# lyd405121/ti-raytrace

Measured on AMD Instinct MI355X. Metric: Mrays/s (primary+secondary) at 1024² 100k-tri, 1/2/4/8 GPU + HBM GB/s, higher is better.
Workload: dtype f32

## Files before the change

### ti_raytrace_amd/csrc/tirt_api.hip

```cpp
#include "tirt_internal.h"
#include "tirt_spectral.h"
#include "tirt_multi_hit.h"
#include <stddef.h>
#include <algorithm>
#include <mutex>
#include <string.h>

namespace tirt {

static thread_local std::string g_error;
void set_error(const std::string &msg) { g_error = msg; }

SceneView scene_view(const tirt_ctx *c)
{
    SceneView s;
    s.vertex = c->vertex.as<float>(); s.primitive = c->primitive.as<int>(); s.material = c->material.as<float>();
    s.shape = c->shape.as<float>(); s.light = c->light.as<int>(); s.env = c->env.as<int>();
    s.mat_lrgb = c->mat_lrgb.as<float>(); s.shade_rec = c->shade_rec.as<float4>(); s.light_rec = c->light_rec.as<float4>();
    s.tex = c->tex_count > 0 ? c->tex.as<int>() : nullptr;
    s.n = c->n; s.light_count = c->light_count; s.env_w = c->env_w; s.env_h = c->env_h; s.env_power = c->env_power;
    return s;
}
BvhView bvh_view(const tirt_ctx *c)
{
// ... 443 lines not shown
    }
    if (!strcmp(name, "plan_batches")) { TIRT_REQUIRE(value >= 0.0 && value <= 64.0, "plan_batches: 0 (automatic) .. 64"); if (flush_pending(c)) return TIRT_ERR_HIP; c->plan_nb = (int)value; return TIRT_OK; }
    if (!strcmp(name, "plan_lanes")) { TIRT_REQUIRE(value >= 0.0 && value <= TIRT_MAX_LANES, "plan_lanes: 0 (automatic) .. the lane count"); if (flush_pending(c)) return TIRT_ERR_HIP; c->plan_lanes = (int)value; return TIRT_OK; }
    if (!strcmp(name, "job_frames")) { TIRT_REQUIRE(value >= 0.0 && value <= 1.0e9, "job_frames out of range"); c->job_frames = (long)value; return TIRT_OK; }
    if (!strcmp(name, "merge_paths")) { TIRT_REQUIRE(value >= 0.0 && value <= 1.0e9, "merge_paths out of range"); c->merge_paths = (size_t)value; c->merge_user = true; return TIRT_OK; }
    if (!strcmp(name, "batch_paths")) {
        TIRT_REQUIRE(value >= 1.0 && value <= 1.0e9, "tirt_set_option: batch_paths out of range");
        c->batch_paths = (size_t)value; c->batch_user = true; return TIRT_OK;
    }
    if (!strcmp(name, "trace_lds_depth")) {
        TIRT_REQUIRE(value >= 12 && value <= 64, "trace_lds_depth: 12..64");
        TIRT_REQUIRE(trace_lds_bytes((int)value) <= c->lds_optin, "trace_lds_depth: stacks + tree top exceed the LDS a block can have on this device");
        c->tr_lds_depth = (int)value; return TIRT_OK;
    }
    if (!strcmp(name, "bdpt_stack_size")) { TIRT_REQUIRE(value >= 16 && value <= 4096, "bdpt_stack_size: 16..4096"); c->bdpt_stack = (int)value; return TIRT_OK; }
    if (!strcmp(name, "trace_timeline")) { c->timeline_arm = (int)value; c->timeline_waves = 0; return TIRT_OK; }
    if (!strcmp(name, "trace_refill_min")) { TIRT_REQUIRE(value >= 1 && value <= 64, "trace_refill_min: 1..64"); c->tr_refill_min = (int)value; return TIRT_OK; }
    if (!strcmp(name, "trace_node_min")) { TIRT_REQUIRE(value >= 1 && value <= 64, "trace_node_min: 1..64"); c->tr_node_min = (int)value; return TIRT_OK; }
    if (!strcmp(name, "bdpt_bounded")) { c->bdpt_bounded = value != 0.0 ? 1 : 0; return TIRT_OK; }
    if (!strcmp(name, "bdpt_state_fill")) { TIRT_REQUIRE(value == 0.0 || value == 1.0 || value == 2.0, "bdpt_state_fill: 0 (none), 1 (zeros) or 2 (poison)"); c->bdpt_state_fill = (int)value; return TIRT_OK; }
    if (!strcmp(name, "primary_beams")) { TIRT_REQUIRE(value == 0.0 || value == 1.0, "primary_beams: 0 or 1"); if (flush_pending(c)) return TIRT_ERR_HIP; c->primary_beams = (int)value; return TIRT_OK; }
    if (!strcmp(name, "primary_beams_rebuild")) { if (flush_pending(c)) return TIRT_ERR_HIP; c->pvb_valid = false; return TIRT_OK; }
    if (!strcmp(name, "primary_beams_diag")) { if (flush_pending(c)) return TIRT_ERR_HIP; c->pvb_diag = value != 0.0; return TIRT_OK; }
    if (!strcmp(name, "primary_beams_min_frames")) { TIRT_REQUIRE(value >= 1.0 && value <= 1.0e6, "primary_beams_min_frames out of range"); if (flush_pending(c)) return TIRT_ERR_HIP; c->primary_beams_min_frames = (int)value; return TIRT_OK; }
    if (!strcmp(name, "bdpt_lanes")) { TIRT_REQUIRE(value >= 1.0 && value <= 4.0, "bdpt_lanes: 1..4"); if (sync_all(c)) return TIRT_ERR_HIP; c->bdpt_lanes = (int)value; return TIRT_OK; }
    if (!strcmp(name, "bdpt_batch_items")) { TIRT_REQUIRE(value >= 1.0 && value <= 1.0e9, "bdpt_batch_items out of range"); c->bdpt_batch_items = (size_t)value; return TIRT_OK; }
    if (!strcmp(name, "bdpt_mem_budget")) { TIRT_REQUIRE(value >= 0, "bdpt_mem_budget: bytes >= 0"); c->bdpt_mem_budget = (size_t)value; return TIRT_OK; }
    if (!strcmp(name, "trace_slices")) {
        const int iv = (int)value;
        TIRT_REQUIRE(iv >= 1 && iv <= 64 && (iv & (iv - 1)) == 0, "trace_slices: power of two, 1..64");
        int l = 0; while ((1 << l) < iv) l++;
        c->tr_slice_log2 = l; return TIRT_OK;
    }
    if (!strcmp(name, "shade_specialize")) { TIRT_REQUIRE(value == 0.0 || value == 1.0, "shade_specialize: 0 (generic kernel) or 1"); if (flush_pending(c)) return TIRT_ERR_HIP; c->shade_specialize = (int)value; return TIRT_OK; }
    if (!strcmp(name, "shade_grid")) { TIRT_REQUIRE(value >= 1 && value <= 65536, "shade_grid: 1..65536"); c->sh_grid = (int)value; c->grid_user = true; return TIRT_OK; }
    if (!strcmp(name, "path_order_blocks")) { c->path_order_blocks = value != 0.0; return TIRT_OK; }
    if (!strcmp(name, "slices_contiguous")) { c->slices_contiguous = value != 0.0; return TIRT_OK; }
    if (!strcmp(name, "trace_grid_alone")) { TIRT_REQUIRE(value >= 1 && value <= 16384, "trace_grid_alone: 1..16384"); c->tr_grid_alone = (int)value; return TIRT_OK; }
    if (!strcmp(name, "query_chunk_rays")) {
        TIRT_REQUIRE(value >= 256.0 && value <= (double)(1 << 27), "query_chunk_rays: 256 .. 2^27");
        c->query_chunk = (size_t)value; return TIRT_OK;
    }
    if (!strcmp(name, "trace_grid")) { TIRT_REQUIRE(value >= 1 && value <= 16384, "trace_grid: 1..16384"); c->tr_grid = (int)value; c->grid_user = true; return TIRT_OK; }
    set_error(std::string("tirt_set_option: unknown option ") + name);
    return TIRT_ERR_ARG;
}
// ... 957 lines not shown
```

### ti_raytrace_amd/csrc/tirt_internal.h

```cpp
#pragma once
#include <hip/hip_runtime.h>
#include <stdint.h>
#include <stdio.h>
#include <initializer_list>
#include <string>
#include <type_traits>
#include <vector>
#include "../../include/tirt.h"
#include "tirt_device.h"

namespace tirt {

void set_error(const std::string &msg);

#define TIRT_HIP(call)                                                                          \
    do {                                                                                        \
        hipError_t e__ = (call);                                                                \
        if (e__ != hipSuccess) {                                                                \
            tirt::set_error(std::string(#call) + ": " + hipGetErrorString(e__));                \
            return TIRT_ERR_HIP;                                                                \
        }                                                                                       \
    } while (0)

#define TIRT_REQUIRE(cond, msg)                                                                 \
// ... 257 lines not shown
    long job_frames = 0;
    struct { bool valid = false; uint32_t begin = 0; int count = 0; uint32_t seed = 0; int max_depth = 0, stack_size = 0, flags = 0; bool spectral = false; } pend;
    int tr_lds_depth = 16, tr_refill_min = 18, tr_node_min = 38, tr_grid = 1280, tr_slice_log2 = 5, sh_grid = 1024;
    int path_order_blocks = 1, slices_contiguous = 0;
    int tr_grid_alone = 1280;
    tirt::DevBuf counters_mem, spill;
    int cu_count = 256;

    tirt::DevBuf bdpt_px;
    struct BdLane { tirt::DevBuf items, state, rays, hits, qidx, ctr, rad; hipEvent_t delta_done = nullptr, film_done = nullptr; } bd[4];
    int bdpt_lanes = 2;
    int bdpt_state_fill = 0;
    size_t bdpt_batch_items = (size_t)16 << 20;
    size_t bdpt_mem_budget = 0;
    int bdpt_stack = 64;
    int bdpt_bounded = 1;

    struct PvbKey { tirt::CameraView cam; unsigned long long build; int W, H, tile_rank, tile_count, tile_size, tile_blocked, P; } pvb_key;
    bool pvb_valid = false; int primary_beams = 1, primary_beams_min_frames = 16;
    unsigned long long build_serial = 0;
    struct PvbSet { tirt::DevBuf count, cand, bound; hipEvent_t busy = nullptr; } pvb_set[2];
    int pvb_cur = 0;
    int pvb_diag = 0;
    std::vector<std::pair<hipEvent_t, hipEvent_t>> pvb_ev;
    unsigned long long pvb_builds = 0, pvb_build_ns = 0, pvb_skipped = 0;
    tirt::DevBuf pvb_stat, pvb_tmp;

    tirt::DevBuf spec_dev;
    tirt::DevBuf spec_mem; bool spec_set = false; void *spec_view = nullptr;

    tirt::DevBuf trace_stage;
    tirt::DevBuf debug_mem;
    tirt::DevBuf query_mem; size_t query_chunk = (size_t)1 << 21;
    hipEvent_t query_ev_in = nullptr, query_ev_out = nullptr;
    tirt::DevBuf sd_tab, sd_state; bool sd_tab_valid = false, sd_tab_checked = false; int sd_tab_stack = 0;
    tirt::DevBuf dyn_mem;

    void *comm = nullptr; int comm_rank = 0, comm_size = 0;

    tirt::DevBuf dev_counters;
    double ms_build = 0, ms_render = 0, ms_trace_closest = 0, ms_trace_shadow = 0, ms_shade = 0;
    uint64_t launches_trace_closest = 0, launches_trace_shadow = 0, launches_shade = 0;
    bool time_kernels = false;
    std::vector<std::pair<hipEvent_t, hipEvent_t>> ev_pool;
};

// ... 148 lines not shown
```

### ti_raytrace_amd/csrc/tirt_pvb.hip

```cpp
#include "tirt_trace.h"
#include <cstring>

namespace tirt {

constexpr int PVB_CMAX = 24;
constexpr int PVB_STACK = 96;
constexpr float PVB_WIDEN = 0.55f;
constexpr float PVB_REACH = 1.5f;
constexpr int PVB_BLOCK = 1024;

struct PvbView { const int *count; const int2 *cand; const float *bound; };

__global__ void k_pvb_probes(CameraView cam, TileMap tm, int P, float4 *rays)
{
    const int k = blockIdx.x * blockDim.x + threadIdx.x;
    if (k >= P) return;
    const int p = local_to_pixel(tm, k), i = p / tm.H, j = p - i * tm.H;
    for (int pr = 0; pr < 5; pr++) {
        const float jx = pr == 0 ? 0.0f : (((pr - 1) & 1) ? 0.5f : -0.5f), jy = pr == 0 ? 0.0f : (((pr - 1) & 2) ? 0.5f : -0.5f);
        const v3 d = camera_ray_direction(cam, i, j, jx, jy);
        const size_t r = (size_t)pr * P + k;
        rays[2 * r] = make_float4(cam.eye[0], cam.eye[1], cam.eye[2], d.x);
        rays[2 * r + 1] = make_float4(d.y, d.z, 0.0f, 0.0f);
    }
}

TD float h2f(unsigned h) { return (float)__builtin_bit_cast(_Float16, (unsigned short)h); }

__global__ __launch_bounds__(64) void k_pvb_beam(BvhView b, CameraView cam, TileMap tm, int P, const float4 *probe_hits, int *count, int2 *cand, float *bound_out,
                                                 unsigned long long *stat)
{
    __shared__ int s_stack[PVB_STACK];
    __shared__ int2 s_list[PVB_CMAX * 64];
    const int lane = threadIdx.x, k = blockIdx.x * 64 + lane;
// ... 113 lines not shown
        }
        for (int a = 0; a < n; a++) cand[(size_t)a * P + k] = s_list[a * 64 + lane];
    }
    if (live) { count[k] = whole ? n : -1; bound_out[k] = bound; }
    if (stat) {
        const unsigned long long m = __ballot(whole);
        unsigned long long sm = whole ? (unsigned long long)n : 0ull;
        for (int o = 32; o > 0; o >>= 1) sm += __shfl_down(sm, o, 64);
        const unsigned long long mb = __ballot(whole && bound < INF_VALUE);
        if (lane == 0) { atomicAdd(&stat[0], (unsigned long long)__popcll(m)); atomicAdd(&stat[1], sm); atomicAdd(&stat[2], (unsigned long long)__popcll(mb)); }
    }
}

__global__ __launch_bounds__(PVB_BLOCK) void k_pvb_cand(BvhView b, PvbView pv, const float *dx, const float *dy, const float *dz, v3 eye, TileMap tm, int P, int S,
                                                  float4 *hit, int *fb_count, int *fb_slot, float *fb_dx, float *fb_dy, float *fb_dz, DevCounters *ctr,
                                                  unsigned long long *stat, unsigned long long *diag)
{
    const int s = blockIdx.x * blockDim.x + threadIdx.x, lane = threadIdx.x & 63;
    const bool live = s < S;
    int k = 0;
    if (tm.F > 0) { const int ch = __builtin_amdgcn_readfirstlane(s >> 6); k = ((ch / tm.F) << 6) | (s & 63); }
    else if (live) { int f; slot_to_frame_pixel(tm, P, s, f, k); }
    const v3 d = live ? V(__builtin_nontemporal_load(&dx[s]), __builtin_nontemporal_load(&dy[s]), __builtin_nontemporal_load(&dz[s])) : V(0.0f, 0.0f, 1.0f);
    const RayCtx r = make_ray(eye, d);
    const bool par = ray_has_parallel_axis(r);
    int n = live ? pv.count[k] : 0;
    const float bound = live ? pv.bound[k] : 0.0f;
    bool resolved = live && n >= 0;
    bool dead = false;
    if (live) {
        float tn;
        if (b.root_qcode >= 0 && !slabs(r, b.root_min[0], b.root_min[1], b.root_min[2], b.root_max[0], b.root_max[1], b.root_max[2], tn)) dead = true;
        if (!((d.x == d.x) & (d.y == d.y) & (d.z == d.z))) dead = true;
    }
    if (dead) { n = 0; resolved = true; }
    if (!resolved) n = 0;
    float hit_t = INF_VALUE, hit_u = 0.0f, hit_v = 0.0f; int hit_prim = -1, hit_leaf = -1;
    int steps = 0, trips = 0;
    for (int c = 0; c < PVB_CMAX; c++) {
        int2 en = make_int2(0, 0x7f800000);
        if (c < n) en = pv.cand[(size_t)c * P + k];
        const bool go = c < n && __int_as_float(en.y) <= hit_t;
        if (!go) n = 0;
        if (__ballot(go) == 0ull) break;
        trips++; if (go) steps++;
        if (go) (void)trace_leaf_step<true>(b, r, par, ~en.x, hit_t, hit_u, hit_v, hit_prim, hit_leaf);
    }
    if (resolved && !dead && !(hit_t <= bound) && bound < INF_VALUE) resolved = false;
    if (resolved) {
        typedef float f4n __attribute__((ext_vector_type(4)));
        f4n hv = {hit_t, hit_u, hit_v, __int_as_float(hit_prim)};
        __builtin_nontemporal_store(hv, (f4n *)&hit[s]);
    }
    const bool fb = live && !resolved;
    const unsigned long long fm = __ballot(fb);
    __shared__ int s_wn[PVB_BLOCK / 64], s_base;
    const int wid = threadIdx.x >> 6;
    if (lane == 0) s_wn[wid] = __popcll(fm);
    __syncthreads();
    if (threadIdx.x == 0) {
        int tot = 0;
#pragma unroll
        for (int w = 0; w < PVB_BLOCK / 64; w++) tot += s_wn[w];
        s_base = tot ? atomicAdd(fb_count, tot) : 0;
        if (stat && tot) atomicAdd(&stat[3], (unsigned long long)tot);
    }
    __syncthreads();
    if (fb) {
        const unsigned long long lt = (lane == 0) ? 0ull : (~0ull >> (64 - lane));
        int at = s_base + __popcll(fm & lt);
        for (int w = 0; w < wid; w++) at += s_wn[w];
// ... 91 lines not shown
```

### ti_raytrace_amd/csrc/tirt_render.hip

```cpp
#include "tirt_trace.h"
#include "tirt_spectral.h"

namespace tirt {

struct ShadeStep {
    bool want_next = false, want_shadow = false, shaded = false, adds = false;
    v3 add = V(0.0f, 0.0f, 0.0f);
    v3 next_o = V(0.0f, 0.0f, 0.0f), next_d = next_o, next_thr = next_o, sh_o = next_o, sh_d = next_o, sh_c = next_o;
    float next_pdf = 0.0f, sh_dist = 0.0f; int next_spec = 0, sh_expect = -2;
};
template <unsigned FEAT, bool LIST = false>
TD void shade_path(const SceneView &sc, const TileMap &tm, int P, uint32_t frame_begin, uint32_t seed, int bounce, int last_bounce, int slot,
                   const v3 origin, const v3 direction, const float4 hrec, v3 throughout, float brdf_pdf, int perfect_spec, ShadeStep &s)
{
    int f, k; slot_to_frame_pixel(tm, P, slot, f, k);
    const uint32_t pixel = (uint32_t)mapped_pixel<LIST>(tm, k);
    const uint32_t frame = frame_begin + (uint32_t)f;
    const uint32_t dim0 = TM_DIM_BOUNCE0 + TM_DIMS_PER_BOUNCE * (uint32_t)bounce;
    const float t = hrec.x;
    constexpr bool ENV_NEE = (FEAT & SF_ENV_SAMPLE) != 0u;
    constexpr bool ENV_HDR = (FEAT & SF_ENV_HDR) != 0u;
    constexpr bool LIGHT_POW = (FEAT & SF_LIGHT_POWER) != 0u;
    [[maybe_unused]] float p_env = 0.0f;
    if constexpr (ENV_NEE) p_env = sc.light_count == 0 ? 1.0f : env_table(sc).share;
// ... 149 lines not shown
    } else if (!(FEAT & SF_ENV)) {
        const float dis = tm_sqrt(direction.x * direction.x + direction.z * direction.z);
        const float big = 3.4028234e38f;
        const bool e_nan = direction.x != direction.x || direction.y != direction.y || direction.z != direction.z ||
                           (absf(direction.x) > big && absf(direction.z) > big) || (absf(direction.y) > big && dis > big);
        const float e1 = e_nan ? tm_nan() : 0.0f;
        s.adds = true; s.add = (V(e1, e1, e1) * throughout) * sc.env_power;
    } else {
        const float dis = tm_sqrt(direction.x * direction.x + direction.z * direction.z);
        const float tx = (tm_atan2(direction.z, direction.x) + PI_SCENE) / PI_SCENE / 2.0f;
        const float ty = tm_atan2(direction.y, dis) / PI_SCENE + 0.5f;
        const v3 e = env_lookup<ENV_HDR>(sc.env, sc.env_w, sc.env_h, tx, ty);
        s.adds = true;
        if constexpr (ENV_NEE) {
            float w = 1.0f;
            if (perfect_spec != 1) w = power_heuristic(brdf_pdf, p_env * env_pdf(env_table(sc), sc.env_w, sc.env_h, direction).pdf);
            s.add = ((e * throughout) * sc.env_power) * w;
        } else
        s.add = (e * throughout) * sc.env_power;
    }
}

template <bool LIST>
__global__ void k_generate(PathSoA ps, CameraView cam, TileMap tm, int P, int S, uint32_t frame_begin, uint32_t seed,
                           DevCounters *ctr)
{
    int s = blockIdx.x * blockDim.x + threadIdx.x;
    if (s >= S) return;
    int f, k; slot_to_frame_pixel(tm, P, s, f, k);
    int p = mapped_pixel<LIST>(tm, k);
    int i = p / tm.H, j = p - i * tm.H;
    uint32_t frame = frame_begin + (uint32_t)f;
    float jx = 0.0f, jy = 0.0f;
    if (frame != 0) {
        jx = tm_rand(seed, (uint32_t)p, frame, TM_DIM_JX) - 0.5f;
        jy = tm_rand(seed, (uint32_t)p, frame, TM_DIM_JY) - 0.5f;
    }
    v3 d = camera_ray_direction(cam, i, j, jx, jy);
    __builtin_nontemporal_store(d.x, &ps.dx[s]); __builtin_nontemporal_store(d.y, &ps.dy[s]); __builtin_nontemporal_store(d.z, &ps.dz[s]);
    if (s == 0) atomicAdd(&ctr->paths, (unsigned long long)S);
}

#ifndef SH_BLOCK
#define SH_BLOCK 256
#endif
#ifndef SH_MIN_WAVES
#define SH_MIN_WAVES 5
#endif
#ifndef SH_MIN_WAVES_NARROW
#define SH_MIN_WAVES_NARROW 5
#endif
#ifndef SH_MIN_WAVES_MAPS
#define SH_MIN_WAVES_MAPS 4
#endif
#ifndef SH_MIN_WAVES_ENV
#define SH_MIN_WAVES_ENV 4
#endif
#ifndef SH_MIN_WAVES_POWER
#define SH_MIN_WAVES_POWER 4
#endif
#ifndef SH_MIN_WAVES_HDR
#define SH_MIN_WAVES_HDR 5
#endif
struct ShadeArgs { PathState ps; PathSoA in, out; };
typedef const __attribute__((address_space(4))) ShadeArgs *cold_shade_t;
#define SH_COLD(ca) cold_shade_t ca = (cold_shade_t)__builtin_amdgcn_kernarg_segment_ptr(); asm volatile("" : "+s"(ca))
#define SH_LD(x) __builtin_nontemporal_load(&(x))
#define SH_ST(x, v) __builtin_nontemporal_store((v), &(x))
template <unsigned FEAT, int MIN_WAVES, bool LIST = false>
__global__ __launch_bounds__(SH_BLOCK, MIN_WAVES) void k_shade(ShadeArgs paths_in_kernarg_segment, SceneView sc, TileMap tm, int P,
                                                   uint32_t frame_begin, uint32_t seed, int bounce, int last_bounce,
                                                   const int *count_ptr, int count_fixed, unsigned long long *append_ctr,
                                                   DevCounters *ctr, v3 eye)
{
    __shared__ unsigned s_wcnt[2][SH_BLOCK / 64];
    __shared__ unsigned long long s_base[2];
    const int lane = threadIdx.x & 63, wid = threadIdx.x >> 6;
    const unsigned long long lt_mask = (lane == 0) ? 0ull : (~0ull >> (64 - lane));
    const int count = count_ptr ? *count_ptr : count_fixed;
    const int total = gridDim.x * blockDim.x;
    const int rounds = (count + total - 1) / total;
    unsigned long long n_shaded = 0;
    for (int it = 0; it < rounds; it++) {
        const int q = it * total + blockIdx.x * blockDim.x + threadIdx.x;
        bool live = q < count, want_next = false, want_shadow = false, adds = false;
// ... 67 lines not shown
            if (first) { SH_ST(f_r[slot], radiance.x); SH_ST(f_g[slot], radiance.y); SH_ST(f_b[slot], radiance.z); }
            else { f_r[slot] = f_r[slot] + radiance.x; f_g[slot] = f_g[slot] + radiance.y; f_b[slot] = f_b[slot] + radiance.z; }
        }
        if (want_shadow) {
            SH_COLD(ca);
            float *const s_ox = ca->ps.sox, *const s_oy = ca->ps.soy, *const s_oz = ca->ps.soz, *const s_dx = ca->ps.sdx, *const s_dy = ca->ps.sdy, *const s_dz = ca->ps.sdz;
            float *const s_cr = ca->ps.scr, *const s_cg = ca->ps.scg, *const s_cb = ca->ps.scb, *const s_dist = ca->ps.sdist;
            int *const s_prim = ca->ps.sprim, *const s_dst = ca->ps.sdst;
            asm volatile("" :: "s"(s_ox), "s"(s_oy), "s"(s_oz), "s"(s_dx), "s"(s_dy), "s"(s_dz), "s"(s_cr), "s"(s_cg), "s"(s_cb), "s"(s_dist), "s"(s_prim), "s"(s_dst));
            SH_ST(s_ox[qs], sh_o.x); SH_ST(s_oy[qs], sh_o.y); SH_ST(s_oz[qs], sh_o.z);
            SH_ST(s_dx[qs], sh_d.x); SH_ST(s_dy[qs], sh_d.y); SH_ST(s_dz[qs], sh_d.z);
            SH_ST(s_cr[qs], sh_c.x); SH_ST(s_cg[qs], sh_c.y); SH_ST(s_cb[qs], sh_c.z);
            SH_ST(s_prim[qs], sh_expect); SH_ST(s_dist[qs], sh_dist);
            SH_ST(s_dst[qs], ~slot);
        }
    }
    __shared__ unsigned long long s_shaded;
    if (threadIdx.x == 0) s_shaded = 0ull;
    __syncthreads();
    n_shaded = wave_sum(n_shaded);
    if ((threadIdx.x & 63) == 0 && n_shaded) atomicAdd(&s_shaded, n_shaded);
    __syncthreads();
    if (threadIdx.x == 0 && s_shaded) atomicAdd(&ctr->shaded, s_shaded);
}

template <bool LIST>
__global__ void k_film(PathState ps, TileMap tm, int P, int F, uint32_t frame_begin, float *hdr)
{
    int k = blockIdx.x * blockDim.x + threadIdx.x;
    if (k >= P) return;
    int p = mapped_pixel<LIST>(tm, k);
    float *px = hdr + (size_t)p * 3;
    float r = px[0], g = px[1], b = px[2];
    for (int f = 0; f < F; f++) {
        int s = frame_pixel_to_slot(tm, P, f, k);
        float frame = (float)(int)(frame_begin + (uint32_t)f);
        float coff = 1.0f / (frame + 1.0f);
        r = __builtin_nontemporal_load(&ps.fr[s]) * coff + r * (1.0f - coff);
        g = __builtin_nontemporal_load(&ps.fg[s]) * coff + g * (1.0f - coff);
        b = __builtin_nontemporal_load(&ps.fb[s]) * coff + b * (1.0f - coff);
    }
    px[0] = r; px[1] = g; px[2] = b;
}

template <unsigned FEAT>
__global__ __launch_bounds__(SH_BLOCK, 4) void k_shade_spec(ShadeArgs paths_in_kernarg_segment, SceneView sc, SpecView sp, TileMap tm, int P,
// ... 201 lines not shown
template <unsigned FEAT, int MIN_WAVES>
__global__ __launch_bounds__(SH_BLOCK, MIN_WAVES) void k_kat_shade_step(SceneView sc, const float *in, int in_stride, float *out, int out_stride, int n)
{
    const int i = blockIdx.x * blockDim.x + threadIdx.x;
    if (i >= n) return;
    const float *a = in + (size_t)i * in_stride;
    float *o = out + (size_t)i * out_stride;
    const TileMap tm = {0, 1, 0x7fffffff, 1, 0, 0};
    v3 radiance = V(a[18], a[19], a[20]);
    ShadeStep ss;
    shade_path<FEAT>(sc, tm, 0x7fffffff, (uint32_t)__float_as_int(a[2]), (uint32_t)__float_as_int(a[0]), __float_as_int(a[3]), __float_as_int(a[4]) != 0, __float_as_int(a[1]),
                     V(a[5], a[6], a[7]), V(a[8], a[9], a[10]), make_float4(a[11], a[12], a[13], a[14]), V(a[15], a[16], a[17]), a[21], __float_as_int(a[22]), ss);
    if (ss.adds) radiance = radiance + ss.add;
    o[0] = radiance.x; o[1] = radiance.y; o[2] = radiance.z; o[3] = __int_as_float(ss.shaded ? 1 : 0); o[4] = __int_as_float(ss.want_next ? 1 : 0);
    o[5] = ss.next_o.x; o[6] = ss.next_o.y; o[7] = ss.next_o.z; o[8] = ss.next_d.x; o[9] = ss.next_d.y; o[10] = ss.next_d.z;
    o[11] = ss.next_thr.x; o[12] = ss.next_thr.y; o[13] = ss.next_thr.z; o[14] = ss.next_pdf; o[15] = __int_as_float(ss.next_spec); o[16] = __int_as_float(ss.want_shadow ? 1 : 0);
    o[17] = ss.sh_o.x; o[18] = ss.sh_o.y; o[19] = ss.sh_o.z; o[20] = ss.sh_d.x; o[21] = ss.sh_d.y; o[22] = ss.sh_d.z;
    o[23] = ss.sh_c.x; o[24] = ss.sh_c.y; o[25] = ss.sh_c.z; o[26] = __int_as_float(ss.sh_expect); o[27] = ss.sh_dist;
}

typedef void (*shade_fn_t)(ShadeArgs, SceneView, TileMap, int, uint32_t, uint32_t, int, int, const int *, int, unsigned long long *, DevCounters *, v3);
typedef void (*shade_spec_fn_t)(ShadeArgs, SceneView, SpecView, TileMap, int, uint32_t, uint32_t, int, int, const int *, int, unsigned long long *, DevCounters *, v3);
typedef void (*kat_step_fn_t)(SceneView, const float *, int, float *, int, int);
struct ShadeInst { unsigned feat; shade_fn_t fn, fn_list; kat_step_fn_t kat; };
struct ShadeSpecInst { unsigned feat; shade_spec_fn_t fn; };
template <unsigned F, int MW>
constexpr ShadeInst shade_inst() { return {F, k_shade<F, MW>, k_shade<F, MW, true>, k_kat_shade_step<F, MW>}; }
constexpr unsigned SF_I_MAPS = SF_ALL | SF_TEXTURE | SF_TEXTURE_PARAM;
constexpr unsigned SF_E = SF_ENV_SAMPLE, SF_H = SF_ENV_HDR, SF_P = SF_LIGHT_POWER;
static const ShadeInst SHADE_RGB[] = {
    shade_inst<SF_LIGHT_SPHERE, SH_MIN_WAVES_NARROW>(),
    shade_inst<SF_LIGHT_TRI, SH_MIN_WAVES_NARROW>(),
    shade_inst<SF_ALL, SH_MIN_WAVES>(),
    shade_inst<SF_ALL | SF_TEXTURE, SH_MIN_WAVES>(),
    shade_inst<SF_I_MAPS, SH_MIN_WAVES_MAPS>(),
    shade_inst<SF_ALL | SF_E, SH_MIN_WAVES_ENV>(), shade_inst<SF_I_MAPS | SF_E, SH_MIN_WAVES_ENV>(),
    shade_inst<SF_ALL | SF_H, SH_MIN_WAVES_HDR>(), shade_inst<SF_I_MAPS | SF_H, SH_MIN_WAVES_MAPS>(),
    shade_inst<SF_ALL | SF_E | SF_H, SH_MIN_WAVES_ENV>(), shade_inst<SF_I_MAPS | SF_E | SF_H, SH_MIN_WAVES_ENV>(),
    shade_inst<SF_ALL | SF_P, SH_MIN_WAVES_POWER>(), shade_inst<SF_I_MAPS | SF_P, SH_MIN_WAVES_MAPS>(),
    shade_inst<SF_ALL | SF_E | SF_P, SH_MIN_WAVES_ENV>(), shade_inst<SF_I_MAPS | SF_E | SF_P, SH_MIN_WAVES_ENV>(),
    shade_inst<SF_ALL | SF_H | SF_P, SH_MIN_WAVES_POWER>(), shade_inst<SF_I_MAPS | SF_H | SF_P, SH_MIN_WAVES_MAPS>(),
    shade_inst<SF_ALL | SF_E | SF_H | SF_P, SH_MIN_WAVES_ENV>(), shade_inst<SF_I_MAPS | SF_E | SF_H | SF_P, SH_MIN_WAVES_ENV>()};
static const ShadeSpecInst SHADE_SPEC_INST[] = {
    {SF_LIGHT_SPHERE, k_shade_spec<SF_LIGHT_SPHERE>}, {SF_LIGHT_TRI, k_shade_spec<SF_LIGHT_TRI>}, {SF_ALL, k_shade_spec<SF_ALL>}};
template <class T, size_t N>
static const T *pick_shade(const T (&tab)[N], unsigned word, int specialize)
{
    for (const T &e : tab)
        if ((e.feat & SF_DERIVED) == (word & SF_DERIVED) && (word & ~SF_CUTOUT & ~e.feat) == 0u && (specialize || (e.feat & SF_ALL) == SF_ALL)) return &e;
    return nullptr;
}
bool shade_instantiation(unsigned word, int specialize, bool spectral, unsigned *feat)
{
    if (spectral) { const ShadeSpecInst *e = pick_shade(SHADE_SPEC_INST, word, specialize); if (e) *feat = e->feat; return e != nullptr; }
    const ShadeInst *e = pick_shade(SHADE_RGB, word, specialize); if (e) *feat = e->feat; return e != nullptr;
}

static kat_step_fn_t kat_step_inst(unsigned feat)
{
    for (const ShadeInst &e : SHADE_RGB) if (e.feat == feat) return e.kat;
// ... 149 lines not shown
    const uint32_t seed = r.seed;
    DevCounters *const ctr = r.ctr;
    hipStream_t st = L.stream;
    TileMap tm = r.tm;
    tm.F = (c->path_order_blocks && (P & 63) == 0) ? F : 0;
    const bool use_beams = r.beams_ready && F >= c->primary_beams_min_frames;
    char *cm = L.counters_mem.as<char>();
    auto append_ctr = [&](int b) { return (unsigned long long *)(cm + LINE * (size_t)b); };
    auto cnt_path = [&](int b) { return (const int *)append_ctr(b - 1); };
    auto cnt_shadow = [&](int b) { return (const int *)append_ctr(b) + 1; };
    auto fetch = [&](int launch) { return (int *)(cm + LINE * (size_t)(max_depth + 1)) + (size_t)launch * TR_FETCH_STRIDE * TR_FETCH_LINES; };
    const ShadeInst *const rgb_inst = spec ? nullptr : pick_shade(SHADE_RGB, shade_word(c), c->shade_specialize);
    const ShadeSpecInst *const spec_inst = spec ? pick_shade(SHADE_SPEC_INST, c->shade_features, c->shade_specialize) : nullptr;
    TIRT_REQUIRE(rgb_inst || spec_inst, "render: no instantiation of the shading kernel serves the scene's feature word " + std::to_string(shade_word(c)) + " (tirt_shade_instantiation)");
    const shade_fn_t shade_fn = !rgb_inst ? nullptr : r.list ? rgb_inst->fn_list : rgb_inst->fn;
    const shade_spec_fn_t shade_spec_fn = spec_inst ? spec_inst->fn : nullptr;

    TIRT_HIP(hipStreamWaitEvent(st, c->ev_main, 0));
    hipEvent_t r0, r1;
    TIRT_HIP(hipEventCreate(&r0)); TIRT_HIP(hipEventCreate(&r1));
    TIRT_HIP(hipEventRecord(r0, st));
    KernelTimers t = {c->time_kernels != 0, st, {}, {}, {}};

    TIRT_HIP(hipMemsetAsync(L.counters_mem.p, 0, lane_counter_bytes(max_depth), st));
    hipLaunchKernelGGL(r.list ? k_generate<true> : k_generate<false>, dim3((S + B - 1) / B), dim3(B), 0, st, L.ps.st[0], c->cam, tm, P, S, f0, seed, ctr);
    bool busy = false;
    if (c->last_film) { busy = hipEventQuery(c->last_film) == hipErrorNotReady; (void)hipGetLastError(); }
    const BatchPlan plan = plan_batches(c);
    const bool two_big = plan.lanes <= 2 && plan.batch >= ((size_t)24 << 20) && !c->grid_user;
    const int grid_cap = (busy && r.n_lanes > 1 && !two_big) ? c->tr_grid : c->tr_grid_alone;
    int grid_full = (S + TR_BLOCK - 1) / TR_BLOCK; if (grid_full > grid_cap) grid_full = grid_cap;
    const int sh_cap = two_big ? 2 * c->sh_grid : c->sh_grid;
    int grid_shade = (S + SH_BLOCK - 1) / SH_BLOCK; if (grid_shade > sh_cap) grid_shade = sh_cap;
    v3 eye_v; eye_v.x = c->cam.eye[0]; eye_v.y = c->cam.eye[1]; eye_v.z = c->cam.eye[2];
    const TraceArgs base = batch_trace_args(c, r, L);
    for (int b = 0; b < max_depth; b++) {
        const PathSoA &in = L.ps.st[b & 1], &out = L.ps.st[(b + 1) & 1];
        TraceArgs a = base;
        a.dx = in.dx; a.dy = in.dy; a.dz = in.dz;
        if (b == 0) for (int k = 0; k < 3; k++) a.eye[k] = c->cam.eye[k];
        else { a.ox = in.ox; a.oy = in.oy; a.oz = in.oz; }
        a.count_ptr = (b == 0) ? nullptr : cnt_path(b); a.count_fixed = S;
        a.scount_ptr = (b == 0) ? nullptr : cnt_shadow(b - 1);
        a.hit = L.ps.hit;
        a.fetch = fetch(b);
        a.rr = in.rr; a.rg = in.rg; a.rb = in.rb;
        if (spec) a.rw = (float *)in.flags;
        a.timeline = timeline_for(c, flags, grid_full);
        const bool beams = b == 0 && use_beams;
        int *const fb_count = (int *)append_ctr(0) + 4;
        float4 *const fb_hit = (float4 *)L.ps.sox;
        if (beams) {
            pvb_launch_cand(c, st, r.bv, in.dx, in.dy, in.dz, tm, P, S, L.ps.hit, fb_count, (int *)out.ox, out.dx, out.dy, out.dz, ctr);
            a.dx = out.dx; a.dy = out.dy; a.dz = out.dz; a.count_ptr = fb_count; a.hit = fb_hit; a.no_ray_count = 1;
        }
        t.begin(t.closest);
        if (int rc = launch_trace(c, st, b == 0 ? KIND_CLOSEST : KIND_MIXED, a, flags, grid_full)) return rc;
        t.end(t.closest);
        if (beams) pvb_launch_scatter(st, fb_count, (const int *)out.ox, fb_hit, L.ps.hit);
        c->launches_trace_closest++;
        if (b == 0 && c->aov.p) { if (int rc = aov_launch(c, L, tm, P, F, f0)) return rc; }

        t.begin(t.shade);
        if (spec)
            hipLaunchKernelGGL(shade_spec_fn, dim3(grid_shade), dim3(SH_BLOCK), 0, st, ShadeArgs{L.ps, in, out}, r.sv, *spec, tm, P, f0, seed, b,
                               (b == max_depth - 1) ? 1 : 0, (b == 0) ? (const int *)nullptr : cnt_path(b), S,
                               append_ctr(b), ctr, eye_v);
        else
        hipLaunchKernelGGL(shade_fn, dim3(grid_shade), dim3(SH_BLOCK), 0, st, ShadeArgs{L.ps, in, out}, r.sv, tm, P, f0, seed, b,
                           (b == max_depth - 1) ? 1 : 0, (b == 0) ? (const int *)nullptr : cnt_path(b), S,
                           append_ctr(b), ctr, eye_v);
        t.end(t.shade);
        c->launches_shade++;

        if (b == max_depth - 1) {
            TraceArgs sa = base;
            sa.ox = L.ps.sox; sa.oy = L.ps.soy; sa.oz = L.ps.soz; sa.dx = L.ps.sdx; sa.dy = L.ps.sdy; sa.dz = L.ps.sdz;
            sa.count_ptr = cnt_shadow(b); sa.count_fixed = 0;
            sa.fetch = fetch(max_depth);
            sa.rr = out.rr; sa.rg = out.rg; sa.rb = out.rb;
            if (spec) sa.rw = (float *)out.flags;
            t.begin(t.shadow);
            if (int rc = launch_trace(c, st, KIND_SHADOW_ACC, sa, flags, grid_full)) return rc;
            t.end(t.shadow);
            c->launches_trace_shadow++;
        }
    }
    if (c->last_film) TIRT_HIP(hipStreamWaitEvent(st, c->last_film, 0));
    if (spec) hipLaunchKernelGGL(k_film_spec, dim3((P + B - 1) / B), dim3(B), 0, st, L.ps, L.ps.fw, *spec, tm, P, F, f0, seed, c->hdr.as<float>());
    else hipLaunchKernelGGL(r.list ? k_film<true> : k_film<false>, dim3((P + B - 1) / B), dim3(B), 0, st, L.ps, tm, P, F, f0, c->hdr.as<float>());
    if (c->mom.p && !spec) { if (int rc = moments_launch(c, L, tm, P, F)) return rc; }
    TIRT_HIP(hipEventRecord(L.film_done, st));
    L.film_recorded = true;
    c->last_film = L.film_done;
    if (use_beams) c->pvb_set[c->pvb_cur].busy = L.film_done;
    TIRT_HIP(hipEventRecord(r1, st));
// ... 40 lines not shown
```

Baseline: 5810.

## Fuse camera ray generation, beam candidate walk and primary shading into one kernel

Adds a fused kernel used on the primary bounce when beams are on. It generates camera directions in-kernel, walks the precomputed beam candidate list, and shades the resolved hits directly. Only unresolved rays are compacted into a fallback list for the full trace, which is followed by a second shade pass. This removes the separate generate, candidate, scatter and shade launches along with their global round-trips of directions and hit records. In exchange it adds a larger kernel with new occupancy bounds and an extra shade launch for the fallback rays.

New measurement: 5928, median of 6. +2.0%, better.

```diff
diff --git a/ti_raytrace_amd/csrc/tirt_api.hip b/ti_raytrace_amd/csrc/tirt_api.hip
--- a/ti_raytrace_amd/csrc/tirt_api.hip
+++ b/ti_raytrace_amd/csrc/tirt_api.hip
@@ -489,6 +489,7 @@
     if (!strcmp(name, "primary_beams")) { TIRT_REQUIRE(value == 0.0 || value == 1.0, "primary_beams: 0 or 1"); if (flush_pending(c)) return TIRT_ERR_HIP; c->primary_beams = (int)value; return TIRT_OK; }
     if (!strcmp(name, "primary_beams_rebuild")) { if (flush_pending(c)) return TIRT_ERR_HIP; c->pvb_valid = false; return TIRT_OK; }
     if (!strcmp(name, "primary_beams_diag")) { if (flush_pending(c)) return TIRT_ERR_HIP; c->pvb_diag = value != 0.0; return TIRT_OK; }
+    if (!strcmp(name, "primary_fused")) { TIRT_REQUIRE(value == 0.0 || value == 1.0, "primary_fused: 0 or 1"); if (flush_pending(c)) return TIRT_ERR_HIP; c->primary_fused = (int)value; return TIRT_OK; }
     if (!strcmp(name, "primary_beams_min_frames")) { TIRT_REQUIRE(value >= 1.0 && value <= 1.0e6, "primary_beams_min_frames out of range"); if (flush_pending(c)) return TIRT_ERR_HIP; c->primary_beams_min_frames = (int)value; return TIRT_OK; }
     if (!strcmp(name, "bdpt_lanes")) { TIRT_REQUIRE(value >= 1.0 && value <= 4.0, "bdpt_lanes: 1..4"); if (sync_all(c)) return TIRT_ERR_HIP; c->bdpt_lanes = (int)value; return TIRT_OK; }
     if (!strcmp(name, "bdpt_batch_items")) { TIRT_REQUIRE(value >= 1.0 && value <= 1.0e9, "bdpt_batch_items out of range"); c->bdpt_batch_items = (size_t)value; return TIRT_OK; }
diff --git a/ti_raytrace_amd/csrc/tirt_internal.h b/ti_raytrace_amd/csrc/tirt_internal.h
--- a/ti_raytrace_amd/csrc/tirt_internal.h
+++ b/ti_raytrace_amd/csrc/tirt_internal.h
@@ -303,6 +303,7 @@
     struct PvbSet { tirt::DevBuf count, cand, bound; hipEvent_t busy = nullptr; } pvb_set[2];
     int pvb_cur = 0;
     int pvb_diag = 0;
+    int primary_fused = 1;
     std::vector<std::pair<hipEvent_t, hipEvent_t>> pvb_ev;
     unsigned long long pvb_builds = 0, pvb_build_ns = 0, pvb_skipped = 0;
     tirt::DevBuf pvb_stat, pvb_tmp;
diff --git a/ti_raytrace_amd/csrc/tirt_pvb.h b/ti_raytrace_amd/csrc/tirt_pvb.h
--- /dev/null
+++ b/ti_raytrace_amd/csrc/tirt_pvb.h
@@ -0,0 +1,41 @@
+#pragma once
+#include "tirt_trace.h"
+
+namespace tirt {
+
+constexpr int PVB_CMAX = 24;
+
+struct PvbView { const int *count; const int2 *cand; const float *bound; };
+
+TD bool pvb_walk_list(const BvhView &b, const PvbView &pv, const int P, const int k, const bool live, const v3 eye, const v3 d,
+                      float &hit_t, float &hit_u, float &hit_v, int &hit_prim, int &steps, int &trips)
+{
+    const RayCtx r = make_ray(eye, d);
+    const bool par = ray_has_parallel_axis(r);
+    int n = live ? pv.count[k] : 0;
+    const float bound = live ? pv.bound[k] : 0.0f;
+    bool resolved = live && n >= 0;
+    bool dead = false;
+    if (live) {
+        float tn;
+        if (b.root_qcode >= 0 && !slabs(r, b.root_min[0], b.root_min[1], b.root_min[2], b.root_max[0], b.root_max[1], b.root_max[2], tn)) dead = true;
+        if (!((d.x == d.x) & (d.y == d.y) & (d.z == d.z))) dead = true;
+    }
+    if (dead) { n = 0; resolved = true; }
+    if (!resolved) n = 0;
+    hit_t = INF_VALUE; hit_u = 0.0f; hit_v = 0.0f; hit_prim = -1;
+    int hit_leaf = -1;
+    for (int c = 0; c < PVB_CMAX; c++) {
+        int2 en = make_int2(0, 0x7f800000);
+        if (c < n) en = pv.cand[(size_t)c * P + k];
+        const bool go = c < n && __int_as_float(en.y) <= hit_t;
+        if (!go) n = 0;
+        if (__ballot(go) == 0ull) break;
+        trips++; if (go) steps++;
+        if (go) (void)trace_leaf_step<true>(b, r, par, ~en.x, hit_t, hit_u, hit_v, hit_prim, hit_leaf);
+    }
+    if (resolved && !dead && !(hit_t <= bound) && bound < INF_VALUE) resolved = false;
+    return resolved;
+}
+
+}
diff --git a/ti_raytrace_amd/csrc/tirt_pvb.hip b/ti_raytrace_amd/csrc/tirt_pvb.hip
--- a/ti_raytrace_amd/csrc/tirt_pvb.hip
+++ b/ti_raytrace_amd/csrc/tirt_pvb.hip
@@ -1,15 +1,12 @@
-#include "tirt_trace.h"
+#include "tirt_pvb.h"
 #include <cstring>
 
 namespace tirt {
 
-constexpr int PVB_CMAX = 24;
 constexpr int PVB_STACK = 96;
 constexpr float PVB_WIDEN = 0.55f;
 constexpr float PVB_REACH = 1.5f;
 constexpr int PVB_BLOCK = 1024;
-
-struct PvbView { const int *count; const int2 *cand; const float *bound; };
 
 __global__ void k_pvb_probes(CameraView cam, TileMap tm, int P, float4 *rays)
 {
@@ -169,31 +166,9 @@
     if (tm.F > 0) { const int ch = __builtin_amdgcn_readfirstlane(s >> 6); k = ((ch / tm.F) << 6) | (s & 63); }
     else if (live) { int f; slot_to_frame_pixel(tm, P, s, f, k); }
     const v3 d = live ? V(__builtin_nontemporal_load(&dx[s]), __builtin_nontemporal_load(&dy[s]), __builtin_nontemporal_load(&dz[s])) : V(0.0f, 0.0f, 1.0f);
-    const RayCtx r = make_ray(eye, d);
-    const bool par = ray_has_parallel_axis(r);
-    int n = live ? pv.count[k] : 0;
-    const float bound = live ? pv.bound[k] : 0.0f;
-    bool resolved = live && n >= 0;
-    bool dead = false;
-    if (live) {
-        float tn;
-        if (b.root_qcode >= 0 && !slabs(r, b.root_min[0], b.root_min[1], b.root_min[2], b.root_max[0], b.root_max[1], b.root_max[2], tn)) dead = true;
-        if (!((d.x == d.x) & (d.y == d.y) & (d.z == d.z))) dead = true;
-    }
-    if (dead) { n = 0; resolved = true; }
-    if (!resolved) n = 0;
-    float hit_t = INF_VALUE, hit_u = 0.0f, hit_v = 0.0f; int hit_prim = -1, hit_leaf = -1;
+    float hit_t, hit_u, hit_v; int hit_prim;
     int steps = 0, trips = 0;
-    for (int c = 0; c < PVB_CMAX; c++) {
-        int2 en = make_int2(0, 0x7f800000);
-        if (c < n) en = pv.cand[(size_t)c * P + k];
-        const bool go = c < n && __int_as_float(en.y) <= hit_t;
-        if (!go) n = 0;
-        if (__ballot(go) == 0ull) break;
-        trips++; if (go) steps++;
-        if (go) (void)trace_leaf_step<true>(b, r, par, ~en.x, hit_t, hit_u, hit_v, hit_prim, hit_leaf);
-    }
-    if (resolved && !dead && !(hit_t <= bound) && bound < INF_VALUE) resolved = false;
+    const bool resolved = pvb_walk_list(b, pv, P, k, live, eye, d, hit_t, hit_u, hit_v, hit_prim, steps, trips);
     if (resolved) {
         typedef float f4n __attribute__((ext_vector_type(4)));
         f4n hv = {hit_t, hit_u, hit_v, __int_as_float(hit_prim)};
diff --git a/ti_raytrace_amd/csrc/tirt_render.hip b/ti_raytrace_amd/csrc/tirt_render.hip
--- a/ti_raytrace_amd/csrc/tirt_render.hip
+++ b/ti_raytrace_amd/csrc/tirt_render.hip
@@ -1,4 +1,4 @@
-#include "tirt_trace.h"
+#include "tirt_pvb.h"
 #include "tirt_spectral.h"
 
 namespace tirt {
@@ -195,11 +195,8 @@
 }
 
 template <bool LIST>
-__global__ void k_generate(PathSoA ps, CameraView cam, TileMap tm, int P, int S, uint32_t frame_begin, uint32_t seed,
-                           DevCounters *ctr)
-{
-    int s = blockIdx.x * blockDim.x + threadIdx.x;
-    if (s >= S) return;
+TD v3 camera_path_direction(const CameraView &cam, const TileMap &tm, int P, int s, uint32_t frame_begin, uint32_t seed)
+{
     int f, k; slot_to_frame_pixel(tm, P, s, f, k);
     int p = mapped_pixel<LIST>(tm, k);
     int i = p / tm.H, j = p - i * tm.H;
@@ -209,7 +206,16 @@
         jx = tm_rand(seed, (uint32_t)p, frame, TM_DIM_JX) - 0.5f;
         jy = tm_rand(seed, (uint32_t)p, frame, TM_DIM_JY) - 0.5f;
     }
-    v3 d = camera_ray_direction(cam, i, j, jx, jy);
+    return camera_ray_direction(cam, i, j, jx, jy);
+}
+
+template <bool LIST>
+__global__ void k_generate(PathSoA ps, CameraView cam, TileMap tm, int P, int S, uint32_t frame_begin, uint32_t seed,
+                           DevCounters *ctr)
+{
+    int s = blockIdx.x * blockDim.x + threadIdx.x;
+    if (s >= S) return;
+    v3 d = camera_path_direction<LIST>(cam, tm, P, s, frame_begin, seed);
     __builtin_nontemporal_store(d.x, &ps.dx[s]); __builtin_nontemporal_store(d.y, &ps.dy[s]); __builtin_nontemporal_store(d.z, &ps.dz[s]);
     if (s == 0) atomicAdd(&ctr->paths, (unsigned long long)S);
 }
@@ -234,6 +240,12 @@
 #endif
 #ifndef SH_MIN_WAVES_HDR
 #define SH_MIN_WAVES_HDR 5
+#endif
+#ifndef SH_MIN_WAVES_FUSED_NARROW
+#define SH_MIN_WAVES_FUSED_NARROW 6
+#endif
+#ifndef SH_MIN_WAVES_FUSED_WIDE
+#define SH_MIN_WAVES_FUSED_WIDE 4
 #endif
 struct ShadeArgs { PathState ps; PathSoA in, out; };
 typedef const __attribute__((address_space(4))) ShadeArgs *cold_shade_t;
@@ -347,6 +359,133 @@
     if ((threadIdx.x & 63) == 0 && n_shaded) atomicAdd(&s_shaded, n_shaded);
     __syncthreads();
     if (threadIdx.x == 0 && s_shaded) atomicAdd(&ctr->shaded, s_shaded);
+}
+
+template <unsigned FEAT, int MIN_WAVES, bool WALK>
+__global__ __launch_bounds__(SH_BLOCK, MIN_WAVES) void k_pvb_cand_shade(ShadeArgs paths_in_kernarg_segment, SceneView sc, BvhView bv, PvbView pv, CameraView cam, TileMap tm, int P,
+                                                            uint32_t frame_begin, uint32_t seed, int last_bounce,
+                                                            const int *count_ptr, int count_fixed, unsigned long long *append_ctr, int *fb_count,
+                                                            DevCounters *ctr, unsigned long long *stat)
+{
+    __shared__ unsigned s_wcnt[2][SH_BLOCK / 64], s_fcnt[2][SH_BLOCK / 64];
+    __shared__ unsigned long long s_base[2];
+    __shared__ int s_fbase[2];
+    const int lane = threadIdx.x & 63, wid = threadIdx.x >> 6;
+    const unsigned long long lt_mask = (lane == 0) ? 0ull : (~0ull >> (64 - lane));
+    const int count = count_ptr ? *count_ptr : count_fixed;
+    const int total = gridDim.x * blockDim.x;
+    const int rounds = (count + total - 1) / total;
+    const v3 eye = V(cam.eye[0], cam.eye[1], cam.eye[2]);
+    unsigned long long n_shaded = 0;
+    for (int it = 0; it < rounds; it++) {
+        const int q = it * total + blockIdx.x * blockDim.x + threadIdx.x;
+        const bool live = q < count;
+        bool shade = false, left = false, want_next = false, want_shadow = false;
+        int slot = 0;
+        v3 direction = V(0.0f, 0.0f, 1.0f);
+        float4 hrec = make_float4(INF_VALUE, 0.0f, 0.0f, __int_as_float(-1));
+        if constexpr (WALK) {
+            int k = 0;
+            if (tm.F > 0) { const int ch = __builtin_amdgcn_readfirstlane(q >> 6); k = ((ch / tm.F) << 6) | (q & 63); }
+            else if (live) { int f; slot_to_frame_pixel(tm, P, q, f, k); }
+            slot = q;
+            if (live) direction = camera_path_direction<false>(cam, tm, P, q, frame_begin, seed);
+            float hit_t, hit_u, hit_v; int hit_prim, steps = 0, trips = 0;
+            shade = pvb_walk_list(bv, pv, P, k, live, eye, direction, hit_t, hit_u, hit_v, hit_prim, steps, trips);
+            hrec = make_float4(hit_t, hit_u, hit_v, __int_as_float(hit_prim));
+            left = live && !shade;
+        } else if (live) {
+            SH_COLD(ca);
+            const int *const c_slot = (const int *)ca->in.ox; const float4 *const c_hit = ca->ps.hit;
+            const float *const c_dx = ca->in.dx, *const c_dy = ca->in.dy, *const c_dz = ca->in.dz;
+            asm volatile("" :: "s"(c_slot), "s"(c_hit), "s"(c_dx), "s"(c_dy), "s"(c_dz));
+            slot = SH_LD(c_slot[q]);
+            direction = V(SH_LD(c_dx[q]), SH_LD(c_dy[q]), SH_LD(c_dz[q]));
+            typedef float f4nt__ __attribute__((ext_vector_type(4)));
+            const f4nt__ hnt__ = __builtin_nontemporal_load((const f4nt__ *)&c_hit[q]);
+            hrec = make_float4(hnt__.x, hnt__.y, hnt__.z, hnt__.w);
+            shade = true;
+        }
+        v3 radiance = V(0.0f, 0.0f, 0.0f), next_o = radiance, next_d = radiance, next_thr = radiance;
+        v3 sh_o = radiance, sh_d = radiance, sh_c = radiance;
+        float next_pdf = 0.0f, sh_dist = 0.0f; int next_spec = 0, sh_expect = -2;
+        if (shade) {
+            ShadeStep ss;
+            shade_path<FEAT, false>(sc, tm, P, frame_begin, seed, 0, last_bounce, slot, eye, direction, hrec, V(1.0f, 1.0f, 1.0f), 1.0f, 1, ss);
+            want_next = ss.want_next; want_shadow = ss.want_shadow; if (ss.shaded) n_shaded++;
+            next_o = ss.next_o; next_d = ss.next_d; next_thr = ss.next_thr; next_pdf = ss.next_pdf; next_spec = ss.next_spec;
+            sh_o = ss.sh_o; sh_d = ss.sh_d; sh_c = ss.sh_c; sh_expect = ss.sh_expect; sh_dist = ss.sh_dist;
+            if (ss.adds) radiance = radiance + ss.add;
+        }
+        const int par = it & 1;
+        const unsigned long long nmask = __ballot(want_next), smask = __ballot(want_shadow), fmask = WALK ? __ballot(left) : 0ull;
+        if (lane == 0) { s_wcnt[par][wid] = (unsigned)__popcll(nmask) | ((unsigned)__popcll(smask) << 16); if (WALK) s_fcnt[par][wid] = (unsigned)__popcll(fmask); }
+        __syncthreads();
+        if (threadIdx.x == 0) {
+            unsigned tn = 0, tsd = 0, tf = 0;
+#pragma unroll
+            for (int w = 0; w < SH_BLOCK / 64; w++) { tn += s_wcnt[par][w] & 0xffffu; tsd += s_wcnt[par][w] >> 16; if (WALK) tf += s_fcnt[par][w]; }
+            s_base[par] = (tn | tsd) ? atomicAdd(append_ctr, (unsigned long long)tn | ((unsigned long long)tsd << 32)) : 0ull;
+            if (WALK) {
+                s_fbase[par] = tf ? atomicAdd(fb_count, (int)tf) : 0;
+                if (stat && tf) atomicAdd(&stat[3], (unsigned long long)tf);
+            }
+        }
+        __syncthreads();
+        unsigned pn = 0, psd = 0, pf = 0;
+#pragma unroll
+        for (int w = 0; w < SH_BLOCK / 64; w++) if (w < wid) { pn += s_wcnt[par][w] & 0xffffu; psd += s_wcnt[par][w] >> 16; if (WALK) pf += s_fcnt[par][w]; }
+        const unsigned long long bb = s_base[par];
+        const int qn = (int)(unsigned)(bb & 0xffffffffull) + (int)pn + __popcll(nmask & lt_mask);
+        const int qs = (int)(unsigned)(bb >> 32) + (int)psd + __popcll(smask & lt_mask);
+        if (WALK && left) {
+            SH_COLD(ca);
+            int *const l_slot = (int *)ca->in.ox; float *const l_dx = ca->in.dx, *const l_dy = ca->in.dy, *const l_dz = ca->in.dz;
+            asm volatile("" :: "s"(l_slot), "s"(l_dx), "s"(l_dy), "s"(l_dz));
+            const int at = s_fbase[par] + (int)pf + __popcll(fmask & lt_mask);
+            l_slot[at] = slot; l_dx[at] = direction.x; l_dy[at] = direction.y; l_dz[at] = direction.z;
+        }
+        if (want_next) {
+            SH_COLD(ca);
+            float *const o_ox = ca->out.ox, *const o_oy = ca->out.oy, *const o_oz = ca->out.oz, *const o_dx = ca->out.dx, *const o_dy = ca->out.dy, *const o_dz = ca->out.dz;
+            float *const o_tr = ca->out.tr, *const o_tg = ca->out.tg, *const o_tb = ca->out.tb;
+            float *const o_pdf = ca->out.brdf_pdf; int *const o_slot = ca->out.slot;
+            asm volatile("" :: "s"(o_ox), "s"(o_oy), "s"(o_oz), "s"(o_dx), "s"(o_dy), "s"(o_dz), "s"(o_tr), "s"(o_tg), "s"(o_tb), "s"(o_pdf), "s"(o_slot));
+            SH_ST(o_ox[qn], next_o.x); SH_ST(o_oy[qn], next_o.y); SH_ST(o_oz[qn], next_o.z);
+            SH_ST(o_dx[qn], next_d.x); SH_ST(o_dy[qn], next_d.y); SH_ST(o_dz[qn], next_d.z);
+            SH_ST(o_tr[qn], next_thr.x); SH_ST(o_tg[qn], next_thr.y); SH_ST(o_tb[qn], next_thr.z);
+            SH_ST(o_pdf[qn], next_pdf); SH_ST(o_slot[qn], (int)((uint32_t)slot | ((uint32_t)next_spec << 31)));
+        }
+        if (shade) {
+            SH_COLD(ca);
+            float *const f_r = ca->ps.fr, *const f_g = ca->ps.fg, *const f_b = ca->ps.fb;
+            asm volatile("" :: "s"(f_r), "s"(f_g), "s"(f_b));
+            SH_ST(f_r[slot], radiance.x); SH_ST(f_g[slot], radiance.y); SH_ST(f_b[slot], radiance.z);
+        }
+        if (want_shadow) {
+            SH_COLD(ca);
+            float *const s_ox = ca->ps.sox, *const s_oy = ca->ps.soy, *const s_oz = ca->ps.soz, *const s_dx = ca->ps.sdx, *const s_dy = ca->ps.sdy, *const s_dz = ca->ps.sdz;
+            float *const s_cr = ca->ps.scr, *const s_cg = ca->ps.scg, *const s_cb = ca->ps.scb, *const s_dist = ca->ps.sdist;
+            int *const s_prim = ca->ps.sprim, *const s_dst = ca->ps.sdst;
+            asm volatile("" :: "s"(s_ox), "s"(s_oy), "s"(s_oz), "s"(s_dx), "s"(s_dy), "s"(s_dz), "s"(s_cr), "s"(s_cg), "s"(s_cb), "s"(s_dist), "s"(s_prim), "s"(s_dst));
+            SH_ST(s_ox[qs], sh_o.x); SH_ST(s_oy[qs], sh_o.y); SH_ST(s_oz[qs], sh_o.z);
+            SH_ST(s_dx[qs], sh_d.x); SH_ST(s_dy[qs], sh_d.y); SH_ST(s_dz[qs], sh_d.z);
+            SH_ST(s_cr[qs], sh_c.x); SH_ST(s_cg[qs], sh_c.y); SH_ST(s_cb[qs], sh_c.z);
+            SH_ST(s_prim[qs], sh_expect); SH_ST(s_dist[qs], sh_dist);
+            SH_ST(s_dst[qs], ~slot);
+        }
+    }
+    __shared__ unsigned long long s_shaded;
+    if (threadIdx.x == 0) s_shaded = 0ull;
+    __syncthreads();
+    n_shaded = wave_sum(n_shaded);
+    if ((threadIdx.x & 63) == 0 && n_shaded) atomicAdd(&s_shaded, n_shaded);
+    __syncthreads();
+    if (threadIdx.x == 0 && s_shaded) atomicAdd(&ctr->shaded, s_shaded);
+    if (WALK && blockIdx.x == 0 && threadIdx.x == 0) {
+        atomicAdd(&ctr->paths, (unsigned long long)count); atomicAdd(&ctr->rays_closest, (unsigned long long)count);
+        if (stat) atomicAdd(&stat[4], (unsigned long long)count);
+    }
 }
 
 template <bool LIST>
@@ -594,20 +733,21 @@
 typedef void (*shade_fn_t)(ShadeArgs, SceneView, TileMap, int, uint32_t, uint32_t, int, int, const int *, int, unsigned long long *, DevCounters *, v3);
 typedef void (*shade_spec_fn_t)(ShadeArgs, SceneView, SpecView, TileMap, int, uint32_t, uint32_t, int, int, const int *, int, unsigned long long *, DevCounters *, v3);
 typedef void (*kat_step_fn_t)(SceneView, const float *, int, float *, int, int);
-struct ShadeInst { unsigned feat; shade_fn_t fn, fn_list; kat_step_fn_t kat; };
+typedef void (*fused_fn_t)(ShadeArgs, SceneView, BvhView, PvbView, CameraView, TileMap, int, uint32_t, uint32_t, int, const int *, int, unsigned long long *, int *, DevCounters *, unsigned long long *);
+struct ShadeInst { unsigned feat; shade_fn_t fn, fn_list; kat_step_fn_t kat; fused_fn_t fused, fused_rest; };
 struct ShadeSpecInst { unsigned feat; shade_spec_fn_t fn; };
-template <unsigned F, int MW>
-constexpr ShadeInst shade_inst() { return {F, k_shade<F, MW>, k_shade<F, MW, true>, k_kat_shade_step<F, MW>}; }
+template <unsigned F, int MW, int MW_WALK = MW>
+constexpr ShadeInst shade_inst() { return {F, k_shade<F, MW>, k_shade<F, MW, true>, k_kat_shade_step<F, MW>, k_pvb_cand_shade<F, MW_WALK, true>, k_pvb_cand_shade<F, MW, false>}; }
 constexpr unsigned SF_I_MAPS = SF_ALL | SF_TEXTURE | SF_TEXTURE_PARAM;
 constexpr unsigned SF_E = SF_ENV_SAMPLE, SF_H = SF_ENV_HDR, SF_P = SF_LIGHT_POWER;
 static const ShadeInst SHADE_RGB[] = {
-    shade_inst<SF_LIGHT_SPHERE, SH_MIN_WAVES_NARROW>(),
-    shade_inst<SF_LIGHT_TRI, SH_MIN_WAVES_NARROW>(),
-    shade_inst<SF_ALL, SH_MIN_WAVES>(),
-    shade_inst<SF_ALL | SF_TEXTURE, SH_MIN_WAVES>(),
+    shade_inst<SF_LIGHT_SPHERE, SH_MIN_WAVES_NARROW, SH_MIN_WAVES_FUSED_NARROW>(),
+    shade_inst<SF_LIGHT_TRI, SH_MIN_WAVES_NARROW, SH_MIN_WAVES_FUSED_NARROW>(),
+    shade_inst<SF_ALL, SH_MIN_WAVES, SH_MIN_WAVES_FUSED_WIDE>(),
+    shade_inst<SF_ALL | SF_TEXTURE, SH_MIN_WAVES, SH_MIN_WAVES_FUSED_WIDE>(),
     shade_inst<SF_I_MAPS, SH_MIN_WAVES_MAPS>(),
     shade_inst<SF_ALL | SF_E, SH_MIN_WAVES_ENV>(), shade_inst<SF_I_MAPS | SF_E, SH_MIN_WAVES_ENV>(),
-    shade_inst<SF_ALL | SF_H, SH_MIN_WAVES_HDR>(), shade_inst<SF_I_MAPS | SF_H, SH_MIN_WAVES_MAPS>(),
+    shade_inst<SF_ALL | SF_H, SH_MIN_WAVES_HDR, SH_MIN_WAVES_FUSED_WIDE>(), shade_inst<SF_I_MAPS | SF_H, SH_MIN_WAVES_MAPS>(),
     shade_inst<SF_ALL | SF_E | SF_H, SH_MIN_WAVES_ENV>(), shade_inst<SF_I_MAPS | SF_E | SF_H, SH_MIN_WAVES_ENV>(),
     shade_inst<SF_ALL | SF_P, SH_MIN_WAVES_POWER>(), shade_inst<SF_I_MAPS | SF_P, SH_MIN_WAVES_MAPS>(),
     shade_inst<SF_ALL | SF_E | SF_P, SH_MIN_WAVES_ENV>(), shade_inst<SF_I_MAPS | SF_E | SF_P, SH_MIN_WAVES_ENV>(),
@@ -803,8 +943,10 @@
     TIRT_HIP(hipEventRecord(r0, st));
     KernelTimers t = {c->time_kernels != 0, st, {}, {}, {}};
 
+    const bool fused = use_beams && c->primary_fused && !spec && !r.list && !c->aov.p && !c->pvb_diag;
+
     TIRT_HIP(hipMemsetAsync(L.counters_mem.p, 0, lane_counter_bytes(max_depth), st));
-    hipLaunchKernelGGL(r.list ? k_generate<true> : k_generate<false>, dim3((S + B - 1) / B), dim3(B), 0, st, L.ps.st[0], c->cam, tm, P, S, f0, seed, ctr);
+    if (!fused) hipLaunchKernelGGL(r.list ? k_generate<true> : k_generate<false>, dim3((S + B - 1) / B), dim3(B), 0, st, L.ps.st[0], c->cam, tm, P, S, f0, seed, ctr);
     bool busy = false;
     if (c->last_film) { busy = hipEventQuery(c->last_film) == hipErrorNotReady; (void)hipGetLastError(); }
     const BatchPlan plan = plan_batches(c);
@@ -831,28 +973,43 @@
         const bool beams = b == 0 && use_beams;
         int *const fb_count = (int *)append_ctr(0) + 4;
         float4 *const fb_hit = (float4 *)L.ps.sox;
-        if (beams) {
+        const bool fuse = beams && fused;
+        auto launch_fused = [&](fused_fn_t fn, const int *count_ptr) {
+            const tirt_ctx::PvbSet &ps = c->pvb_set[c->pvb_cur];
+            t.begin(t.shade);
+            hipLaunchKernelGGL(fn, dim3(grid_shade), dim3(SH_BLOCK), 0, st, ShadeArgs{L.ps, in, out}, r.sv, r.bv, PvbView{ps.count.as<int>(), ps.cand.as<int2>(), ps.bound.as<float>()},
+                               c->cam, tm, P, f0, seed, (max_depth == 1) ? 1 : 0, count_ptr, S, append_ctr(0), fb_count, ctr, c->pvb_stat.as<unsigned long long>());
+            t.end(t.shade);
+            c->launches_shade++;
+        };
+        if (fuse) {
+            launch_fused(rgb_inst->fused, nullptr);
+            a.count_ptr = fb_count; a.no_ray_count = 1;
+        } else if (beams) {
             pvb_launch_cand(c, st, r.bv, in.dx, in.dy, in.dz, tm, P, S, L.ps.hit, fb_count, (int *)out.ox, out.dx, out.dy, out.dz, ctr);
             a.dx = out.dx; a.dy = out.dy; a.dz = out.dz; a.count_ptr = fb_count; a.hit = fb_hit; a.no_ray_count = 1;
         }
         t.begin(t.closest);
         if (int rc = launch_trace(c, st, b == 0 ? KIND_CLOSEST : KIND_MIXED, a, flags, grid_full)) return rc;
         t.end(t.closest);
-        if (beams) pvb_launch_scatter(st, fb_count, (const int *)out.ox, fb_hit, L.ps.hit);
+        if (beams && !fuse) pvb_launch_scatter(st, fb_count, (const int *)out.ox, fb_hit, L.ps.hit);
         c->launches_trace_closest++;
         if (b == 0 && c->aov.p) { if (int rc = aov_launch(c, L, tm, P, F, f0)) return rc; }
 
-        t.begin(t.shade);
-        if (spec)
-            hipLaunchKernelGGL(shade_spec_fn, dim3(grid_shade), dim3(SH_BLOCK), 0, st, ShadeArgs{L.ps, in, out}, r.sv, *spec, tm, P, f0, seed, b,
-                               (b == max_depth - 1) ? 1 : 0, (b == 0) ? (const int *)nullptr : cnt_path(b), S,
-                               append_ctr(b), ctr, eye_v);
-        else
-        hipLaunchKernelGGL(shade_fn, dim3(grid_shade), dim3(SH_BLOCK), 0, st, ShadeArgs{L.ps, in, out}, r.sv, tm, P, f0, seed, b,
-                           (b == max_depth - 1) ? 1 : 0, (b == 0) ? (const int *)nullptr : cnt_path(b), S,
-                           append_ctr(b), ctr, eye_v);
-        t.end(t.shade);
-        c->launches_shade++;
+        if (fuse) launch_fused(rgb_inst->fused_rest, fb_count);
+        else {
+            t.begin(t.shade);
+            if (spec)
+                hipLaunchKernelGGL(shade_spec_fn, dim3(grid_shade), dim3(SH_BLOCK), 0, st, ShadeArgs{L.ps, in, out}, r.sv, *spec, tm, P, f0, seed, b,
+                                   (b == max_depth - 1) ? 1 : 0, (b == 0) ? (const int *)nullptr : cnt_path(b), S,
+                                   append_ctr(b), ctr, eye_v);
+            else
+                hipLaunchKernelGGL(shade_fn, dim3(grid_shade), dim3(SH_BLOCK), 0, st, ShadeArgs{L.ps, in, out}, r.sv, tm, P, f0, seed, b,
+                                   (b == max_depth - 1) ? 1 : 0, (b == 0) ? (const int *)nullptr : cnt_path(b), S,
+                                   append_ctr(b), ctr, eye_v);
+            t.end(t.shade);
+            c->launches_shade++;
+        }
 
         if (b == max_depth - 1) {
             TraceArgs sa = base;
```
